# mrluin/TextualDegRemoval

Hardware: AMD Instinct MI355X
Metric: train images/sec (512x512, bs=4/GPU) (higher is better)
Workload: dtype f32 (3xbf16-split MFMA: 24-bit operand significands on the full fp32 exponent range, fp32 accumulate; unscaled gradients, no loss scale, no step-skip guard; tensors fp32 -- the MASA-encoder ResidualBlock activations / gradients as three bf16 planes whose sum IS the fp32 value, bit for bit)

## Files before the change

### include/tdr.h

```cpp
#ifndef TDR_H
#define TDR_H
#include <stdint.h>
#ifdef __cplusplus
extern "C" {
#endif

#define TDR_ABI_VERSION 112
int tdr_version(void);
const char* tdr_last_error(void);

typedef struct TdrStepGuard {
    float scale, inv_scale, max_scale;
    int good, growth_interval;
    int step, skipped, finite;
    float bc1, bc2_sqrt;
} TdrStepGuard;

typedef struct TdrConvDesc {
    int N, Cin, H, W;
    int Cout, OH, OW;
    int KH, stride, dil, pad;
    const float* in;  int64_t in_ns;
    int gate;
    const float* kscale; int64_t kscale_ns;
// ... 69 lines not shown
int64_t tdr_wgrad3x3_p16_ws_floats(const TdrWgradP16Desc* d);
int tdr_wgrad3x3_p16(const TdrWgradP16Desc* d, void* stream);

typedef struct TdrWgradDesc {
    int N, Cin, H, W, Cout, OH, OW, KH, stride, pad;
    const float* in;   int64_t in_ns;  int gate;
    const float* dout; int64_t dout_ns;
    float* g;
    float* db;
    int per_image;
    float* ws; int64_t ws_floats;
    int math;
} TdrWgradDesc;
int64_t tdr_wgrad_ws_floats(const TdrWgradDesc* d);
int tdr_conv_wgrad(const TdrWgradDesc* d, void* stream);

typedef struct TdrWg1GroupEntry {
    const float* in; const float* dout; float* part; float* dbpart; float* g; float* db;
} TdrWg1GroupEntry;
int tdr_wgrad1x1_group_supported(const TdrWgradDesc* d);
int64_t tdr_wgrad1x1_group_ws_floats(const TdrWgradDesc* d, int nprob);
int tdr_wgrad1x1_group(const TdrWgradDesc* d, int nprob, const void* table, void* stream);

int64_t tdr_wgrad3x3_p16_group_ws_floats(const TdrWgradP16Desc* d, int nprob);
int tdr_wgrad3x3_p16_group_plan(const TdrWgradP16Desc* d, int nprob, int* nsplit, int* units, int* units_per_wg);
int tdr_wgrad3x3_p16_group(const TdrWgradP16Desc* d, int nprob, const void* table, void* stream);

int tdr_layernorm2d_fwd(const float* x, int64_t x_ns, const float* w, const float* b, float eps, int center,
                        int N, int C, int HW, float* y, float* mu, float* rstd, void* stream);
int64_t tdr_ln_ws_floats(int N, int C, int HW);
// ... 36 lines not shown
int tdr_mdta_pad(int C);
int tdr_mdta_softmax(const float* G, const float* ss, const float* temp, int N, int C, int heads, float* A, float* AT,
                     void* stream);
int tdr_mdta_bwd(const float* G, const float* ss, const float* temp, const float* A, const float* dA, int N, int C,
                 int heads, float* W, float* dtemp, float* ws, void* stream);
int tdr_attn_fold_proj(const float* AT, const float* Wo, int N, int C, int heads, float* Wf, void* stream);
int tdr_axpby_dev(const float* a, const float* alpha, const float* b, int64_t numel, float* out, void* stream);
int tdr_dot(const float* a, const float* b, int64_t numel, float* out, float* ws, void* stream);
int tdr_pixel_shuffle2(const float* in, int N, int C, int H, int W, float* out, void* stream);

int tdr_sca_fwd(const float* pooled, const float* wsca, const float* bsca, int N, int C, float* s, void* stream);
int tdr_sca_bwd(const float* G3, const float* S3, const float* w3, const float* b3, const float* beta,
                const float* s, const float* pooled, const float* wsca, int N, int C,
                float* dw3, float* db3, float* dbeta, float* dwsca, float* dbsca, float* dpooled,
                float* ws , void* stream);
int tdr_scaled_conv_param_grads(const float* G, const float* S, const float* w, const float* b,
                                const float* gamma, int Cout, int Cin, float* dw, float* db, float* dgamma,
                                void* stream);

int64_t tdr_chansum_ws_floats(int N, int C, int HW);
int tdr_channel_sum(const float* x, int64_t x_ns, int N, int C, int HW, float* out, float* ws, void* stream);

int tdr_copy_rows(const float* src, int64_t src_ns, float* dst, int64_t dst_ns, int N, int64_t len, void* stream);
int tdr_add_rows(const float* src, int64_t src_ns, float* dst, int64_t dst_ns, int N, int64_t len, void* stream);
int tdr_pixel_unshuffle2(const float* in, int N, int C, int H, int W, float* out, void* stream);
int tdr_pad_crop(const float* src, int N, int C, int Hs, int Ws, float* dst, int Hd, int Wd, void* stream);
int tdr_crop_augment(const float* src, int64_t src_ns, int N, int C, int Hs, int Ws, const int* top, const int* left,
                     const int* mode, const float* noise, const float* sigma, int P, float* out, void* stream);

int64_t tdr_ssim3d_ws_floats(int H, int W);
// ... 363 lines not shown
```

### textualdegremoval_amd/csrc/tdr_pointwise.hip

```cpp
#include "tdr_common.h"
#include "../../include/tdr.h"

namespace {

template <int SLICES, int CPT>
__global__ __launch_bounds__(64 * SLICES) void ln_fwd_kernel(const float* __restrict__ x, long x_ns,
                                                            const float* __restrict__ w, const float* __restrict__ b,
                                                            float eps, int center, int C, int HW,
                                                            float* __restrict__ y, float* __restrict__ mu,
                                                            float* __restrict__ rstd) {
    __shared__ float red[SLICES][64];
    const int lane = threadIdx.x & 63, slice = threadIdx.x >> 6;
    const int px = blockIdx.x * 64 + lane, n = blockIdx.y;
    const bool pok = px < HW;
    const float* xn = x + (long)n * x_ns + (pok ? px : HW - 1);
    float v[CPT];
    float s = 0.f;
#pragma unroll
    for (int i = 0; i < CPT; ++i) v[i] = xn[(long)min(slice + SLICES * i, C - 1) * HW];
#pragma unroll
    for (int i = 0; i < CPT; ++i) {
        v[i] = (pok && slice + SLICES * i < C) ? v[i] : 0.f;
        s += v[i];
    }
// ... 546 lines not shown
            if (n == 0) {
                float sb = 0.f;
                for (int m = 0; m < N; ++m) sb += ds[(long)m * C + cj];
                dbsca[cj] = sb;
            }
        }
        return;
    }
    const int colb = (C + 255) / 256;
    const int r = (int)blockIdx.x - ntail;
    const int ci = (r / colb) * 4 + (threadIdx.x >> 8), cj = (r % colb) * 256 + (threadIdx.x & 255);
    if (ci >= C || cj >= C) return;
    float a = 0.f;
    for (int n = 0; n < N; ++n) a += ds[(long)n * C + ci] * pooled[(long)n * C + cj];
    dwsca[(long)ci * C + cj] = a;
}

__global__ __launch_bounds__(256) void scaled_conv_param_kernel(const float* __restrict__ G, const float* __restrict__ S,
                                                               const float* __restrict__ w, const float* __restrict__ b,
                                                               const float* __restrict__ gamma, int Cin,
                                                               float* __restrict__ dw, float* __restrict__ db,
                                                               float* __restrict__ dgamma) {
    __shared__ float red[4];
    const int co = blockIdx.x;
    const float gm = gamma[co];
    float acc = 0.f;
    for (int ci = threadIdx.x; ci < Cin; ci += 256) {
        const float gv = G[(long)co * Cin + ci];
        dw[(long)co * Cin + ci] = gm * gv;
        acc += w[(long)co * Cin + ci] * gv;
// ... 376 lines not shown
        hipLaunchKernelGGL(sca_bwd_rows_kernel, dim3(C), dim3(256), 0, st, G3, S3, w3, b3, beta, s, N, C, dw3, db3, dbeta);
        hipLaunchKernelGGL(sca_bwd_ds_kernel, dim3(tdr_cdiv(C, 64), N), dim3(1024), 0, st, G3, w3, beta, N, C, ds);
        hipLaunchKernelGGL(sca_bwd_dw_kernel, dim3(tdr_cdiv(C, 256), C), dim3(256), 0, st, ds, pooled, N, C, dwsca);
        hipLaunchKernelGGL(sca_bwd_tail_kernel, dim3(tdr_cdiv(C, 64), N), dim3(1024), 0, st, ds, wsca, N, C, dbsca, dpooled);
    } else {
        const int nt = tdr_cdiv(C, 64) * N;
        hipLaunchKernelGGL(sca_bwd_a_kernel, dim3(nt + tdr_cdiv(C, 4)), dim3(1024), 0, st, G3, S3, w3, b3, beta, s, N, C, nt, dw3,
                           db3, dbeta, ds);
        hipLaunchKernelGGL(sca_bwd_b_kernel, dim3(nt + tdr_cdiv(C, 4) * tdr_cdiv(C, 256)), dim3(1024), 0, st, ds, pooled, wsca, N, C,
                           nt, dwsca, dbsca, dpooled);
    }
    TDR_LAUNCH_CHECK("sca_bwd");
    return TDR_OK;
}

extern "C" int tdr_scaled_conv_param_grads(const float* G, const float* S, const float* w, const float* b,
                                           const float* gamma, int Cout, int Cin, float* dw, float* db, float* dgamma,
                                           void* stream) {
    TDR_REQUIRE(G && S && w && b && gamma && dw && db && dgamma, "tdr_scaled_conv_param_grads: null pointer");
    hipLaunchKernelGGL(scaled_conv_param_kernel, dim3(Cout), dim3(256), 0, (hipStream_t)stream, G, S, w, b, gamma, Cin, dw,
                       db, dgamma);
    TDR_LAUNCH_CHECK("scaled_conv_param_kernel");
    return TDR_OK;
}

extern "C" int64_t tdr_chansum_ws_floats(int N, int C, int HW) {
    (void)N; (void)HW;
    return (int64_t)C * CS_SPLITS;
}

// ... 164 lines not shown
```

### textualdegremoval_amd/csrc/tdr_wgrad_1x1.hip

```cpp
#include "tdr_common.h"
#include "tdr_wgrad_common.h"
#include "../../include/tdr.h"
#include <stdlib.h>

typedef __bf16 g1bf16x8 __attribute__((ext_vector_type(8)));
typedef _Float16 g1f16x8 __attribute__((ext_vector_type(8)));
typedef unsigned g1u32x4 __attribute__((ext_vector_type(4)));

namespace {

enum { G1_BX3 = 0, G1_HX2 = 1 };

constexpr int G1_PX = 32;

template <int SCH>
__device__ __forceinline__ void g1_split8(const f32x4& a, const f32x4& b, g1u32x4 (&p)[SCH == G1_BX3 ? 3 : 2]) {
    if constexpr (SCH == G1_BX3) {
        unsigned h[4], m[4], l[4];
        tdr_split3_bf16<false>(a[0], a[1], h[0], m[0], l[0]);
        tdr_split3_bf16<false>(a[2], a[3], h[1], m[1], l[1]);
        tdr_split3_bf16<false>(b[0], b[1], h[2], m[2], l[2]);
        tdr_split3_bf16<false>(b[2], b[3], h[3], m[3], l[3]);
        p[0] = (g1u32x4){h[0], h[1], h[2], h[3]};
        p[1] = (g1u32x4){m[0], m[1], m[2], m[3]};
// ... 179 lines not shown
    constexpr size_t lds = (size_t)RING * (BM + (GATE ? 2 : 1) * BN) * 128;
    static_assert(lds <= 160 * 1024, "LDS");
    dim3 grid(N * a.spi, tdr_cdiv(a.Cout, BM), tdr_cdiv(a.Cin, BN));
    auto kern = wgrad1x1_dma_kernel<TMW, TNW, GATE, SCH, RING>;
    static bool attr_set = false;
    if (!attr_set) {
        (void)hipFuncSetAttribute(reinterpret_cast<const void*>(kern), hipFuncAttributeMaxDynamicSharedMemorySize, 160 * 1024);
        attr_set = true;
    }
    hipLaunchKernelGGL(kern, grid, dim3(256), lds, st, a);
    TDR_LAUNCH_CHECK("wgrad1x1_dma_kernel");
    return TDR_OK;
}


template <bool GATE, int SCH, int KQ, bool GRP = false, int TNW = 2, int TMW = 2>
__global__ __launch_bounds__(256 * KQ) void wgrad1x1_sp_kernel(WgArgs a) {
    static_assert(KQ == 1 || TMW == 2, "the in-block K split is built for 128-row tiles");
    constexpr int BM = 64 * TMW, BN = 64 * TNW, NI = TMW + TNW;
    constexpr int NS = SCH == G1_BX3 ? 3 : 2, NP = SCH == G1_BX3 ? 6 : 3;
    constexpr int ROWS = BM + BN;
    constexpr int PLANE = ROWS * 32;
    constexpr int KSTR = NS * PLANE + 64;
    constexpr int BUF = KQ * KSTR;
    constexpr int PXS = 16 * KQ;
    constexpr int NL = GATE ? NI + TNW : NI;

    extern __shared__ __attribute__((aligned(1024))) unsigned char smem_raw[];
    const int tid = threadIdx.x, lane = tid & 63, wave = __builtin_amdgcn_readfirstlane(tid >> 6);
    const int kq = KQ == 2 ? wave >> 2 : 0, wm = (wave >> 1) & 1, wn = wave & 1;
    const int j = lane & 31, kg = lane >> 5;

    int prob = 0, split = blockIdx.x, by = blockIdx.y, bz = blockIdx.z;
// ... 136 lines not shown
        split_store(raw0, 0, s + 2 < nst);
        interleave();
        __syncthreads();
    }

    if (want_db) {
#pragma unroll
        for (int i = 0; i < TMW; ++i) {
            float t = dsum[i];
            t += __shfl_xor(t, 1, 64); t += __shfl_xor(t, 2, 64);
            if constexpr (KQ == 2) t += __shfl_xor(t, 4, 64);
            const int co = co0 + lr + 64 * i;
            if (lp == 0 && co < a.Cout) a.dbpart[(long)split * a.Cout + co] = t;
        }
    }
    float* red = reinterpret_cast<float*>(smem_raw);
    const int wq = wave & 3;
    if (KQ == 2 && kq == 1) {
#pragma unroll
        for (int x = 0; x < TMW; ++x)
#pragma unroll
            for (int y = 0; y < TNW; ++y)
#pragma unroll
                for (int r = 0; r < 16; ++r) red[((wq * 4 + x * 2 + y) * 16 + r) * 64 + lane] = acc[x][y][r];
    }
    if constexpr (KQ == 2) {
        __syncthreads();
        if (kq == 1) return;
    }
    float* part = a.part + (long)split * a.Cout * a.Cin;
// ... 11 lines not shown
        }
}

template <bool GATE, int SCH, int KQ>
int launch_sp(const WgArgs& a, int N, hipStream_t st) {
    constexpr int NS = SCH == G1_BX3 ? 3 : 2;
    constexpr size_t lds0 = (size_t)2 * KQ * (NS * 256 * 32 + 64);
    constexpr size_t lds = (KQ == 2 && lds0 < 65536) ? 65536 : lds0;
    dim3 grid(N * a.spi, tdr_cdiv(a.Cout, 128), tdr_cdiv(a.Cin, 128));
    auto kern = wgrad1x1_sp_kernel<GATE, SCH, KQ>;
    static bool attr_set = false;
    if (!attr_set) {
        (void)hipFuncSetAttribute(reinterpret_cast<const void*>(kern), hipFuncAttributeMaxDynamicSharedMemorySize, 160 * 1024);
        attr_set = true;
    }
    hipLaunchKernelGGL(kern, grid, dim3(256 * KQ), lds, st, a);
    TDR_LAUNCH_CHECK("wgrad1x1_sp_kernel");
    return TDR_OK;
}

int g1_sp() {
    static const int v = tdr_tune_env("TDR_WG1_SP") ? atoi(tdr_tune_env("TDR_WG1_SP")) : 2;
    return v;
}

int g1_ring() {
    static const int r = tdr_tune_env("TDR_WG1_RING") ? atoi(tdr_tune_env("TDR_WG1_RING")) : 2;
    return r == 3 ? 3 : 2;
}

template <int TMW, int TNW, int SCH>
int launch_g1_gr(const WgArgs& a, const TdrWgradDesc* d, hipStream_t st) {
// ... 49 lines not shown

template <bool GATE, int SCH, int TNW, int TMW>
int launch_grp(const WgArgs& a, int nprob, hipStream_t st) {
    constexpr int NS = SCH == G1_BX3 ? 3 : 2;
    constexpr size_t lds0 = (size_t)2 * (NS * (64 * TMW + 64 * TNW) * 32 + 64);
    static const size_t pad = tdr_tune_env("TDR_WG1_GRP_LDS") ? (size_t)atol(tdr_tune_env("TDR_WG1_GRP_LDS")) : 0;
    const size_t lds = lds0 < pad ? pad : lds0;
    const int T = a.tiles_x * a.tiles_y;
    dim3 grid((unsigned)tdr_cdiv(a.grp_pairs, 8) * 8 * T);
    auto kern = wgrad1x1_sp_kernel<GATE, SCH, 1, true, TNW, TMW>;
    static bool attr_set = false;
    if (!attr_set) {
        (void)hipFuncSetAttribute(reinterpret_cast<const void*>(kern), hipFuncAttributeMaxDynamicSharedMemorySize, 160 * 1024);
        attr_set = true;
    }
    hipLaunchKernelGGL(kern, grid, dim3(256), lds, st, a);
    TDR_LAUNCH_CHECK("wgrad1x1_sp_kernel<grouped>");
    return TDR_OK;
}

}

extern "C" int tdr_wgrad1x1_group_supported(const TdrWgradDesc* d) {
    if (!d || (d->math != 1 && d->math != 2) || d->per_image) return 0;
    if (d->KH != 1 || d->stride != 1 || d->pad != 0 || d->H != d->OH || d->W != d->OW) return 0;
    const long HW = (long)d->OH * d->OW;
    if (HW % G1_PX != 0 || d->in_ns % 4 != 0 || d->dout_ns % 4 != 0) return 0;
    return d->Cin >= 64 && d->Cout > 64;
}

extern "C" int64_t tdr_wgrad1x1_group_ws_floats(const TdrWgradDesc* d, int nprob) {
// ... 70 lines not shown

int tdr_wgrad_1x1_launch(const WgArgs& a, const WgPlan& p, const TdrWgradDesc* d, hipStream_t st) {
    if (p.cfg == 0 && g1_sp() == 1) {
        const bool g = d->gate != 0;
        if (a.scheme == 1) return g ? launch_sp<true, G1_HX2, 2>(a, d->N, st) : launch_sp<false, G1_HX2, 2>(a, d->N, st);
        return g ? launch_sp<true, G1_BX3, 2>(a, d->N, st) : launch_sp<false, G1_BX3, 2>(a, d->N, st);
    }
    if (p.cfg == 0 && g1_sp() == 2) {
        const bool g = d->gate != 0;
        if (a.scheme == 1) return g ? launch_sp<true, G1_HX2, 1>(a, d->N, st) : launch_sp<false, G1_HX2, 1>(a, d->N, st);
        return g ? launch_sp<true, G1_BX3, 1>(a, d->N, st) : launch_sp<false, G1_BX3, 1>(a, d->N, st);
    }
    if (a.scheme == 1) return p.cfg == 0 ? launch_g1_gr<2, 2, G1_HX2>(a, d, st) : launch_g1_gr<1, 1, G1_HX2>(a, d, st);
    return p.cfg == 0 ? launch_g1_gr<2, 2, G1_BX3>(a, d, st) : launch_g1_gr<1, 1, G1_BX3>(a, d, st);
}
```

### textualdegremoval_amd/csrc/tdr_wgrad_common.h

```cpp
#pragma once
#include "tdr_common.h"

struct TdrWgradDesc;

struct WgArgs {
    const float* in; long in_ns; int Cin, H, W; long gate_off;
    const float* dout; long dout_ns; int Cout, OH, OW;
    int pad, tw_log2, tiles_x, tiles_y, tpi , tps , spi ;
    float* part;
    float* dbpart;
    int scheme;
    const void* grp_tab;
    int grp_bpp;
    int grp_pairs;
};

struct WgPlan { int tw_log2, tiles_x, tiles_y, tpi, tps, spi, cfg, WKw, BMc, BNc; };

bool tdr_wgrad_bx3_supported(const TdrWgradDesc* d);
WgPlan tdr_wgrad_bx3_plan(const TdrWgradDesc* d);
int tdr_wgrad_bx3_launch(const WgArgs& a, const WgPlan& p, const TdrWgradDesc* d, hipStream_t st);

bool tdr_wgrad_s2_supported(const TdrWgradDesc* d);
WgPlan tdr_wgrad_s2_plan(const TdrWgradDesc* d);
int tdr_wgrad_s2_launch(const WgArgs& a, const WgPlan& p, const TdrWgradDesc* d, hipStream_t st);

bool tdr_wgrad_1x1_supported(const TdrWgradDesc* d);
WgPlan tdr_wgrad_1x1_plan(const TdrWgradDesc* d);
int tdr_wgrad_1x1_launch(const WgArgs& a, const WgPlan& p, const TdrWgradDesc* d, hipStream_t st);
```

### textualdegremoval_amd/csrc/tdr_wgrad_mfma.hip

```cpp
#include <stdio.h>
#include <stdlib.h>
#include "tdr_common.h"
#include "tdr_wgrad_common.h"
#include "../../include/tdr.h"

namespace {

constexpr int wg_plane(int TW, int KH, int S) { return (((64 / TW) - 1) * S + KH) * ((TW - 1) * S + KH); }
constexpr int wg_cmax(int a, int b) { return a > b ? a : b; }
constexpr int wg_max_plane(int KH, int S) {
    return wg_cmax(wg_plane(8, KH, S), wg_cmax(wg_plane(16, KH, S), wg_plane(32, KH, S)));
}

template <int KH, int S, int WMw, int WNw, int WKw, int TMW, int TNW, bool GATE>
__global__ __launch_bounds__(256) void wgrad_mfma_kernel(WgArgs a) {
    static_assert(WMw * WNw * WKw == 4, "4 waves");
    constexpr int TAPS = KH * KH;
    constexpr int BMc = 32 * TMW * WMw, BNc = 32 * TNW * WNw;
    constexpr int MAXPIT = (wg_max_plane(KH, S) + 63) / 64;
    constexpr int DPT = BMc / 4;
    constexpr int IPT = BNc / 4;
    constexpr int KPW = 32 / WKw;

    extern __shared__ __attribute__((aligned(16))) float smem[];
// ... 217 lines not shown
    const int TW = 1 << a.tw_log2;
    const int LH = ((64 >> a.tw_log2) - 1) * S + KH, LW = (TW - 1) * S + KH;
    const size_t lds = (size_t)(BMc * 65 + BNc * ((LH * LW) | 1)) * sizeof(float);
    dim3 grid(N * p.spi, tdr_cdiv(a.Cout, BMc), tdr_cdiv(a.Cin, BNc));
    auto kern = wgrad_mfma_kernel<KH, S, WMw, WNw, WKw, TMW, TNW, GATE>;
    static bool attr_set = false;
    if (!attr_set) {
        (void)hipFuncSetAttribute(reinterpret_cast<const void*>(kern), hipFuncAttributeMaxDynamicSharedMemorySize, 160 * 1024);
        attr_set = true;
    }
    hipLaunchKernelGGL(kern, grid, dim3(256), lds, st, a);
    TDR_LAUNCH_CHECK("wgrad_mfma_kernel");
    return TDR_OK;
}

}

extern "C" int64_t tdr_wgrad_ws_floats(const TdrWgradDesc* d) {
    const WgPlan p = make_plan(d);
    return (int64_t)d->N * p.spi * p.WKw * d->Cout * d->Cin * d->KH * d->KH + (int64_t)d->N * p.spi * d->Cout;
}

extern "C" int tdr_conv_wgrad(const TdrWgradDesc* d, void* stream) {
    TDR_REQUIRE(d && d->in && d->dout && d->g && d->ws, "tdr_conv_wgrad: null pointer");
    const WgPlan p = make_plan(d);
    const int64_t need = tdr_wgrad_ws_floats(d);
    TDR_REQUIRE(d->ws_floats >= need, "tdr_conv_wgrad: workspace too small (%lld < %lld)", (long long)d->ws_floats,
                (long long)need);
    WgArgs a;
    a.in = d->in; a.in_ns = d->in_ns; a.Cin = d->Cin; a.H = d->H; a.W = d->W;
    a.gate_off = (long)d->Cin * d->H * d->W;
    a.dout = d->dout; a.dout_ns = d->dout_ns; a.Cout = d->Cout; a.OH = d->OH; a.OW = d->OW;
    a.grp_tab = nullptr; a.grp_bpp = 0; a.grp_pairs = 0;
    a.pad = d->pad; a.tw_log2 = p.tw_log2; a.tiles_x = p.tiles_x; a.tiles_y = p.tiles_y; a.tpi = p.tpi; a.tps = p.tps; a.spi = p.spi;
    const bool direct = !d->db && (d->per_image ? p.spi : d->N * p.spi) * p.WKw == 1;
    a.part = direct ? d->g : d->ws;
    a.dbpart = d->db ? d->ws + (int64_t)d->N * p.spi * p.WKw * d->Cout * d->Cin * d->KH * d->KH : nullptr;
    hipStream_t st = (hipStream_t)stream;
    const bool g = d->gate != 0;
    int rc = TDR_ERR_UNSUPPORTED;
    const int key = d->KH * 10 + d->stride;
    a.scheme = d->math == 3 ? 2 : (d->math == 2 ? 1 : 0);
    static const bool dbg = tdr_tune_env("TDR_WG_DEBUG") != nullptr;
    if (dbg && !(d->math >= 1 && tdr_wgrad_bx3_supported(d)) && !tdr_wgrad_s2_supported(d))
        fprintf(stderr, "[tdr] exact wgrad: math %d N %d %d->%d @%dx%d k%d s%d pad %d gate %d per_image %d in_ns %ld dout_ns %ld\n", d->math,
                d->N, d->Cin, d->Cout, d->H, d->W, d->KH, d->stride, d->pad, d->gate, d->per_image, (long)d->in_ns, (long)d->dout_ns);
    if (tdr_wgrad_1x1_supported(d)) {
        rc = tdr_wgrad_1x1_launch(a, p, d, st);
    } else if (d->math >= 1 && tdr_wgrad_bx3_supported(d)) {
        rc = tdr_wgrad_bx3_launch(a, p, d, st);
    } else if (tdr_wgrad_s2_supported(d)) {
        rc = tdr_wgrad_s2_launch(a, p, d, st);
    } else if (key == 11) {
        switch (p.cfg) {
            case 0: rc = g ? launch_wg<1, 1, 2, 2, 1, 2, 2, true>(a, p, d->N, st) : launch_wg<1, 1, 2, 2, 1, 2, 2, false>(a, p, d->N, st); break;
            case 1: rc = g ? launch_wg<1, 1, 1, 1, 4, 2, 1, true>(a, p, d->N, st) : launch_wg<1, 1, 1, 1, 4, 2, 1, false>(a, p, d->N, st); break;
            case 2: rc = g ? launch_wg<1, 1, 2, 2, 1, 1, 1, true>(a, p, d->N, st) : launch_wg<1, 1, 2, 2, 1, 1, 1, false>(a, p, d->N, st); break;
            default: rc = g ? launch_wg<1, 1, 1, 1, 4, 1, 1, true>(a, p, d->N, st) : launch_wg<1, 1, 1, 1, 4, 1, 1, false>(a, p, d->N, st); break;
        }
    } else if (key == 31 && !g) {
        rc = p.cfg == 3 ? launch_wg<3, 1, 1, 1, 4, 1, 1, false>(a, p, d->N, st) : launch_wg<3, 1, 2, 2, 1, 1, 1, false>(a, p, d->N, st);
    } else if (key == 32 && !g) {
        rc = launch_wg<3, 2, 2, 2, 1, 1, 1, false>(a, p, d->N, st);
    } else if (key == 22 && !g) {
        rc = launch_wg<2, 2, 2, 2, 1, 1, 1, false>(a, p, d->N, st);
    } else {
        tdr_set_error("tdr_conv_wgrad: unsupported (KH=%d stride=%d gate=%d)", d->KH, d->stride, d->gate);
        return TDR_ERR_UNSUPPORTED;
    }
    if (rc != TDR_OK || direct) return rc;
    const long elems = (long)d->Cout * d->Cin * d->KH * d->KH;
    const int groups = d->per_image ? d->N : 1;
    const int per_group = (d->per_image ? p.spi : d->N * p.spi) * p.WKw;
    const int nb_main = tdr_cdiv(elems, 64);
    const int nb2 = d->db ? tdr_cdiv(d->Cout, 64) : 0;
    const int pg2 = d->N * p.spi;
    const dim3 rgrid(nb_main + nb2, groups);
    if (per_group <= 8 && pg2 <= 8)
        hipLaunchKernelGGL(wgrad_reduce_kernel<1>, rgrid, dim3(64), 0, st, d->ws, elems, per_group, d->g, nb_main, a.dbpart,
                           (long)d->Cout, pg2, d->db);
    else if (per_group <= 64 && pg2 <= 64)
        hipLaunchKernelGGL(wgrad_reduce_kernel<4>, rgrid, dim3(256), 0, st, d->ws, elems, per_group, d->g, nb_main, a.dbpart,
                           (long)d->Cout, pg2, d->db);
    else
        hipLaunchKernelGGL(wgrad_reduce_kernel<16>, rgrid, dim3(1024), 0, st, d->ws, elems, per_group, d->g, nb_main, a.dbpart,
                           (long)d->Cout, pg2, d->db);
    TDR_LAUNCH_CHECK("wgrad_reduce_kernel");
    return TDR_OK;
}
```

### textualdegremoval_amd/engine.py

```python
import contextlib
import os
import types

import torch

from . import kernels as K
from . import leaves as L
from .kernels import (EPI_GATEBWD, EPI_PSHUF, PACK_DGRAD_2X2S2, PACK_DGRAD_3X3S2, PACK_DGRAD_S1, PACK_FWD)

LN_EPS = 1e-6
FUSE_TAIL = True
FUSE_HEAD = True
FUSE_CONV3_DGRAD = True
INFER_KERNELS = True
LOCAL_KERNELS = True


def _sub(P, pre):
    n = len(pre)
    return {k[n:]: v for k, v in P.items() if k.startswith(pre)}


def _put(G, pre, g):
    for k, v in g.items():
        G[pre + k] = v


DEFER_WGRAD = True
# ... 105 lines not shown
        else:
            dy, dt4, gw2, gb2 = K.naf_tail_bwd(dout, gamma, t4, y, mu2, rs2, P['norm2.weight'], w5t, w4t, defer_finish=late)
        if late:
            L.leaf_fin(('norm2.weight', 'norm2.bias'), gw2, G)
        else:
            G['norm2.weight'], G['norm2.bias'] = gw2, gb2
    else:
        wp, mp, *_ = K.pack_weights(P['conv5.weight'][:c_out], PACK_DGRAD_S1)
        dt4 = K.conv_forward(dout, wp, mp, c, 1, epi=EPI_GATEBWD, kscale=gamma, aux=t4)
    L.leaf_wgrad1x1((yn, dt4), (yn, dt4, 2 * c, c, False),
                    lambda g4, b4: {'conv4.weight': g4.view(2 * c, c, 1, 1), 'conv4.bias': b4}, G)
    if not fused:
        wp, mp, *_ = K.pack_weights(P['conv4.weight'], PACK_DGRAD_S1)
        dyn = K.conv_forward(dt4, wp, mp, c, 1)
        dy, G['norm2.weight'], G['norm2.bias'] = K.layernorm2d_bwd(dyn, y, mu2, rs2, P['norm2.weight'], add=dout)
    G3, S3 = K.conv_wgrad(g, dy, c, c, 1, per_image=True, want_db=True)
    dw3, db3, dbeta, dwsca, dbsca, dpooled = K.sca_bwd(G3, S3, P['conv3.weight'], P['conv3.bias'], beta, s, pooled,
                                                       P['sca.1.weight'])
    G['conv3.weight'], G['conv3.bias'], G['beta'] = dw3, db3, dbeta
    G['sca.1.weight'], G['sca.1.bias'] = dwsca, dbsca
    if fused and FUSE_CONV3_DGRAD:
        dt1, gdw, gdb = K.dwsg_bwd(dgp, t1, P['conv2.weight'], P['conv2.bias'], dg_bias=dpooled, dg_bias_mul=1.0 / (H * W),
                                   defer_finish=late)
    else:
        wp, mp, *_ = K.pack_weights(P['conv3.weight'], PACK_DGRAD_S1)
        dg = K.conv_forward(dy, wp, mp, c, 1, kscale=beta, scale=s, bias2=dpooled, bias2_mul=1.0 / (H * W))
        dt1, gdw, gdb = K.dwsg_bwd(dg, t1, P['conv2.weight'], P['conv2.bias'], defer_finish=late)
    if isinstance(gdw, K.Finisher):
        L.leaf_fin(('conv2.weight', 'conv2.bias'), gdw, G)
    else:
        G['conv2.weight'], G['conv2.bias'] = gdw, gdb
    L.leaf_wgrad1x1((xn, dt1), (xn, dt1, 2 * c, c, False),
                    lambda g1, b1: {'conv1.weight': g1.view(2 * c, c, 1, 1), 'conv1.bias': b1}, G)
    if FUSE_TAIL and K.naf_tail_supported(c, H * W) and _dgrad_fused_ok() and x.is_contiguous() and dy.is_contiguous():
# ... 537 lines not shown
```

### textualdegremoval_amd/kernels.py

```python
import contextlib
import ctypes as C
import os

import torch

from . import _lib
from ._lib import TdrConvDesc, TdrConvP16Desc, TdrWgradDesc, TdrWgradP16Desc, check

EPI_STD, EPI_GATEBWD, EPI_PSHUF = 0, 1, 2
PACK_FWD, PACK_DGRAD_S1, PACK_DGRAD_2X2S2, PACK_DGRAD_3X3S2 = 0, 1, 2, 3

MATH = os.environ.get('TDR_MATH', 'bx3')
WGRAD_1X1_BX3 = True
FMT_F32, FMT_BX3, FMT_HX2, FMT_H1 = 0, 1, 2, 3


def fp16_path():
    return MATH in ('hx2', 'h1')


GRAD_SCALED = False
BACKWARD_PHASE = False


# ... 549 lines not shown
    d.g = g.data_ptr()
    db = torch.empty(Cout, dtype=torch.float32, device=x.device) if want_db else None
    d.db = _p(db)
    d.per_image = 1 if per_image else 0
    if fp16_path() and (fp16_range or GRAD_SCALED) and (KH == 3 or WGRAD_1X1_BX3):
        d.math = 2 if MATH == 'hx2' else 3
    else:
        d.math = 1 if (MATH != 'f32' and (KH == 3 or WGRAD_1X1_BX3)) else 0
    if _survey is not None and d.math >= 2:
        _survey.probe(dout, 'fwd' if fp16_range else 'grad')
    need = lib.tdr_wgrad_ws_floats(C.byref(d))
    ws = workspace(need, x.device, 'wgrad')
    d.ws, d.ws_floats = ws.data_ptr(), ws.numel()
    check(lib.tdr_conv_wgrad(C.byref(d), _stream()), 'tdr_conv_wgrad')
    return (g, db) if want_db else g


def _wgrad1x1_desc(x, dout, Cout, Cin, gate):
    N, _, H, W = x.shape
    d = TdrWgradDesc()
    d.N, d.Cin, d.H, d.W, d.Cout, d.OH, d.OW = N, Cin, H, W, Cout, H, W
    d.KH, d.stride, d.pad = 1, 1, 0
    d.in_ns, d.gate, d.dout_ns = _dense_nchw(x), 1 if gate else 0, _dense_nchw(dout)
    d.per_image = 0
    if fp16_path() and GRAD_SCALED and WGRAD_1X1_BX3:
        d.math = 2 if MATH == 'hx2' else 3
    else:
        d.math = 1 if (MATH != 'f32' and WGRAD_1X1_BX3) else 0
    return d

# ... 434 lines not shown
    N, Cc = s.shape
    dev = s.device
    dw3 = torch.empty(Cc, Cc, 1, 1, dtype=torch.float32, device=dev)
    db3 = torch.empty(Cc, dtype=torch.float32, device=dev)
    dbeta = torch.empty(1, Cc, 1, 1, dtype=torch.float32, device=dev)
    dwsca = torch.empty(Cc, Cc, 1, 1, dtype=torch.float32, device=dev)
    dbsca = torch.empty(Cc, dtype=torch.float32, device=dev)
    dpooled = torch.empty(N, Cc, dtype=torch.float32, device=dev)
    ws = torch.empty(N * Cc, dtype=torch.float32, device=dev)
    check(lib.tdr_sca_bwd(G3.data_ptr(), S3.data_ptr(), w3.data_ptr(), b3.data_ptr(), beta.data_ptr(), s.data_ptr(),
                          pooled.data_ptr(), wsca.data_ptr(), N, Cc, dw3.data_ptr(), db3.data_ptr(), dbeta.data_ptr(),
                          dwsca.data_ptr(), dbsca.data_ptr(), dpooled.data_ptr(), ws.data_ptr(), _stream()), 'tdr_sca_bwd')
    return dw3, db3, dbeta, dwsca, dbsca, dpooled


def scaled_conv_param_grads(G, S, w, b, gamma):
    lib = _lib.load()
    Cout, Cin = G.shape[-2], G.shape[-1]
    dev = G.device
    dw = torch.empty(Cout, Cin, dtype=torch.float32, device=dev)
    db = torch.empty(Cout, dtype=torch.float32, device=dev)
    dg = torch.empty(Cout, dtype=torch.float32, device=dev)
    check(lib.tdr_scaled_conv_param_grads(G.data_ptr(), S.data_ptr(), w.data_ptr(), b.data_ptr(), gamma.data_ptr(), Cout,
                                          Cin, dw.data_ptr(), db.data_ptr(), dg.data_ptr(), _stream()),
          'tdr_scaled_conv_param_grads')
    return dw, db, dg


def channel_sum(x):
    lib = _lib.load()
# ... 1388 lines not shown
```

Before: 61.89.

## Fold SCA ds into conv3 Gram wgrad epilogue and defer Gram reduction

The per-image 1x1 conv3 weight-gradient kernel gains an epilogue that forms partial ds sums (beta·w3·Gram tile) directly from its accumulators. A new SCA backward kernel then reduces those partials into ds, dwsca, dbsca and dpooled without waiting for the full Gram reduction. The Gram reduce and the conv3/beta parameter-gradient kernels move into a deferred leaf finisher, taking them off the critical path of the activation-gradient chain. The cost is extra register and LDS work in the wgrad epilogue, an extra partials buffer and an added kernel variant.

```diff
diff --git a/include/tdr.h b/include/tdr.h
--- a/include/tdr.h
+++ b/include/tdr.h
@@ -107,6 +107,10 @@
 } TdrWgradDesc;
 int64_t tdr_wgrad_ws_floats(const TdrWgradDesc* d);
 int tdr_conv_wgrad(const TdrWgradDesc* d, void* stream);
+int tdr_wgrad_gram_ds_supported(const TdrWgradDesc* d);
+int tdr_wgrad_gram_ds_parts(const TdrWgradDesc* d);
+int tdr_wgrad_gram_ds(const TdrWgradDesc* d, const float* w3, const float* beta, float* dspart, void* stream);
+int tdr_wgrad_gram_finish(const TdrWgradDesc* d, void* stream);
 
 typedef struct TdrWg1GroupEntry {
     const float* in; const float* dout; float* part; float* dbpart; float* g; float* db;
@@ -173,6 +177,10 @@
                 const float* s, const float* pooled, const float* wsca, int N, int C,
                 float* dw3, float* db3, float* dbeta, float* dwsca, float* dbsca, float* dpooled,
                 float* ws , void* stream);
+int tdr_sca_bwd_parts(const float* dspart, int nk, const float* pooled, const float* wsca, int N, int C, float* ds,
+                      float* dwsca, float* dbsca, float* dpooled, void* stream);
+int tdr_sca_bwd_rows(const float* G3, const float* S3, const float* w3, const float* b3, const float* beta, const float* s,
+                     int N, int C, float* dw3, float* db3, float* dbeta, void* stream);
 int tdr_scaled_conv_param_grads(const float* G, const float* S, const float* w, const float* b,
                                 const float* gamma, int Cout, int Cin, float* dw, float* db, float* dgamma,
                                 void* stream);
diff --git a/textualdegremoval_amd/csrc/tdr_pointwise.hip b/textualdegremoval_amd/csrc/tdr_pointwise.hip
--- a/textualdegremoval_amd/csrc/tdr_pointwise.hip
+++ b/textualdegremoval_amd/csrc/tdr_pointwise.hip
@@ -584,6 +584,82 @@
     float a = 0.f;
     for (int n = 0; n < N; ++n) a += ds[(long)n * C + ci] * pooled[(long)n * C + cj];
     dwsca[(long)ci * C + cj] = a;
+}
+
+__device__ __forceinline__ float sca_fold_run(const float* __restrict__ p, int C, int k0, int k1) {
+    float t = 0.f;
+    for (int k = k0; k < k1; k += 8) {
+        float v[8];
+#pragma unroll
+        for (int u = 0; u < 8; ++u) v[u] = k + u < k1 ? p[(long)(k + u) * C] : 0.f;
+#pragma unroll
+        for (int u = 0; u < 8; ++u) t += v[u];
+    }
+    return t;
+}
+
+constexpr int SCA_PARTS_MAXC = 1024;
+
+__global__ __launch_bounds__(1024) void sca_bwd_bp_kernel(const float* __restrict__ dspart, int nk, int G, int kper,
+                                                         const float* __restrict__ pooled, const float* __restrict__ wsca, int N, int C,
+                                                         int ntail, float* __restrict__ ds, float* __restrict__ dwsca,
+                                                         float* __restrict__ dbsca, float* __restrict__ dpooled) {
+    __shared__ float red[16][64];
+    __shared__ float runs[SCA_PARTS_MAXC];
+    __shared__ float dsl[SCA_PARTS_MAXC];
+    const int tid = threadIdx.x;
+    if ((int)blockIdx.x < ntail) {
+        const int tiles = (C + 63) / 64;
+        const int tile = blockIdx.x % tiles, n = blockIdx.x / tiles;
+        const int g = tid / C, ci = tid - g * C;
+        if (g < G) runs[tid] = sca_fold_run(dspart + (long)n * nk * C + ci, C, g * kper, min(nk, (g + 1) * kper));
+        __syncthreads();
+        if (tid < C) {
+            float t = 0.f;
+            for (int q = 0; q < G; ++q) t += runs[q * C + tid];
+            dsl[tid] = t;
+            if (tile == 0) ds[(long)n * C + tid] = t;
+        }
+        __syncthreads();
+        const int lane = tid & 63, sl = tid >> 6;
+        const int cj = tile * 64 + lane;
+        const int cjc = min(cj, C - 1);
+        float a = 0.f;
+        for (int c = sl; c < C; c += 16) a += wsca[(long)c * C + cjc] * dsl[c];
+        red[sl][lane] = a;
+        __syncthreads();
+        if (sl == 0 && cj < C) {
+            float t = 0.f;
+#pragma unroll
+            for (int q = 0; q < 16; ++q) t += red[q][lane];
+            dpooled[(long)n * C + cj] = t;
+        }
+        return;
+    }
+    const int colb = (C + 255) / 256;
+    const int r = (int)blockIdx.x - ntail;
+    const int ci0 = (r / colb) * 4, sub = tid >> 8;
+    if (tid < 4 * N * G) {
+        const int v = tid / G, g = tid - v * G;
+        const int cic = min(ci0 + v / N, C - 1);
+        runs[tid] = sca_fold_run(dspart + (long)(v % N) * nk * C + cic, C, g * kper, min(nk, (g + 1) * kper));
+    }
+    __syncthreads();
+    if (tid < 4 * N) {
+        float t = 0.f;
+        for (int q = 0; q < G; ++q) t += runs[tid * G + q];
+        dsl[tid] = t;
+    }
+    __syncthreads();
+    const int ci = ci0 + sub, cj = (r % colb) * 256 + (tid & 255);
+    if (ci >= C || cj >= C) return;
+    float a = 0.f, sb = 0.f;
+    for (int n = 0; n < N; ++n) {
+        a += dsl[sub * N + n] * pooled[(long)n * C + cj];
+        sb += dsl[sub * N + n];
+    }
+    dwsca[(long)ci * C + cj] = a;
+    if (cj == 0) dbsca[ci] = sb;
 }
 
 __global__ __launch_bounds__(256) void scaled_conv_param_kernel(const float* __restrict__ G, const float* __restrict__ S,
@@ -990,6 +1066,30 @@
     return TDR_OK;
 }
 
+extern "C" int tdr_sca_bwd_parts(const float* dspart, int nk, const float* pooled, const float* wsca, int N, int C, float* ds,
+                                 float* dwsca, float* dbsca, float* dpooled, void* stream) {
+    TDR_REQUIRE(dspart && pooled && wsca && ds && dwsca && dbsca && dpooled, "tdr_sca_bwd_parts: null pointer");
+    TDR_REQUIRE(nk > 0 && N > 0 && N <= 256 && C > 0 && C <= SCA_PARTS_MAXC, "tdr_sca_bwd_parts: need 0 < N <= 256, 0 < C <= %d, nk > 0", SCA_PARTS_MAXC);
+    int G = SCA_PARTS_MAXC / C;
+    if (G > 256 / N) G = 256 / N;
+    if (G > nk) G = nk;
+    const int kper = tdr_cdiv(nk, G);
+    const int nt = tdr_cdiv(C, 64) * N;
+    hipLaunchKernelGGL(sca_bwd_bp_kernel, dim3(nt + tdr_cdiv(C, 4) * tdr_cdiv(C, 256)), dim3(1024), 0, (hipStream_t)stream, dspart, nk, G, kper,
+                       pooled, wsca, N, C, nt, ds, dwsca, dbsca, dpooled);
+    TDR_LAUNCH_CHECK("sca_bwd_parts");
+    return TDR_OK;
+}
+
+extern "C" int tdr_sca_bwd_rows(const float* G3, const float* S3, const float* w3, const float* b3, const float* beta, const float* s,
+                                int N, int C, float* dw3, float* db3, float* dbeta, void* stream) {
+    TDR_REQUIRE(G3 && S3 && w3 && b3 && beta && s && dw3 && db3 && dbeta, "tdr_sca_bwd_rows: null pointer");
+    hipLaunchKernelGGL(sca_bwd_a_kernel, dim3(tdr_cdiv(C, 4)), dim3(1024), 0, (hipStream_t)stream, G3, S3, w3, b3, beta, s, N, C, 0, dw3, db3,
+                       dbeta, static_cast<float*>(nullptr));
+    TDR_LAUNCH_CHECK("sca_bwd_rows");
+    return TDR_OK;
+}
+
 extern "C" int tdr_scaled_conv_param_grads(const float* G, const float* S, const float* w, const float* b,
                                            const float* gamma, int Cout, int Cin, float* dw, float* db, float* dgamma,
                                            void* stream) {
diff --git a/textualdegremoval_amd/csrc/tdr_wgrad_1x1.hip b/textualdegremoval_amd/csrc/tdr_wgrad_1x1.hip
--- a/textualdegremoval_amd/csrc/tdr_wgrad_1x1.hip
+++ b/textualdegremoval_amd/csrc/tdr_wgrad_1x1.hip
@@ -217,9 +217,10 @@
 }
 
 
-template <bool GATE, int SCH, int KQ, bool GRP = false, int TNW = 2, int TMW = 2>
-__global__ __launch_bounds__(256 * KQ) void wgrad1x1_sp_kernel(WgArgs a) {
+template <bool GATE, int SCH, int KQ, bool GRP = false, int TNW = 2, int TMW = 2, bool DSP = false>
+__global__ __launch_bounds__(256 * KQ) void wgrad1x1_sp_kernel(WgArgs a, G1DsArgs e) {
     static_assert(KQ == 1 || TMW == 2, "the in-block K split is built for 128-row tiles");
+    static_assert(!DSP || (KQ == 1 && !GRP && !GATE && TNW == 2 && TMW == 2), "the ds-partial epilogue: plain 128 x 128 tiles, no in-block K split");
     constexpr int BM = 64 * TMW, BN = 64 * TNW, NI = TMW + TNW;
     constexpr int NS = SCH == G1_BX3 ? 3 : 2, NP = SCH == G1_BX3 ? 6 : 3;
     constexpr int ROWS = BM + BN;
@@ -386,6 +387,36 @@
             if (lp == 0 && co < a.Cout) a.dbpart[(long)split * a.Cout + co] = t;
         }
     }
+    if constexpr (DSP) {
+        float* fold = reinterpret_cast<float*>(smem_raw);
+        float* bl = fold + 256;
+        if (tid < 128) bl[tid] = co0 + tid < a.Cout ? e.beta[co0 + tid] : 0.f;
+        float wv[TNW][TMW][16];
+#pragma unroll
+        for (int y = 0; y < TNW; ++y) {
+            const int cic = min(ci0 + (wn * TNW + y) * 32 + j, a.Cin - 1);
+#pragma unroll
+            for (int x = 0; x < TMW; ++x)
+#pragma unroll
+                for (int r = 0; r < 16; ++r) {
+                    const int co = min(co0 + (wm * TMW + x) * 32 + (r & 3) + 8 * (r >> 2) + 4 * kg, a.Cout - 1);
+                    wv[y][x][r] = *reinterpret_cast<const float*>(reinterpret_cast<const char*>(e.w3) + 4u * (unsigned)(co * a.Cin + cic));
+                }
+        }
+        __syncthreads();
+#pragma unroll
+        for (int y = 0; y < TNW; ++y) {
+            float t = 0.f;
+#pragma unroll
+            for (int x = 0; x < TMW; ++x)
+#pragma unroll
+                for (int r = 0; r < 16; ++r) t += bl[(wm * TMW + x) * 32 + (r & 3) + 8 * (r >> 2) + 4 * kg] * wv[y][x][r] * acc[x][y][r];
+            t += __shfl_xor(t, 32, 64);
+            if (kg == 0) fold[wm * 128 + (wn * TNW + y) * 32 + j] = t;
+        }
+        __syncthreads();
+        if (tid < 128 && ci0 + tid < a.Cin) e.dspart[((long)split * gridDim.y + by) * a.Cin + ci0 + tid] = fold[tid] + fold[128 + tid];
+    }
     float* red = reinterpret_cast<float*>(smem_raw);
     const int wq = wave & 3;
     if (KQ == 2 && kq == 1) {
@@ -427,8 +458,24 @@
         (void)hipFuncSetAttribute(reinterpret_cast<const void*>(kern), hipFuncAttributeMaxDynamicSharedMemorySize, 160 * 1024);
         attr_set = true;
     }
-    hipLaunchKernelGGL(kern, grid, dim3(256 * KQ), lds, st, a);
+    hipLaunchKernelGGL(kern, grid, dim3(256 * KQ), lds, st, a, G1DsArgs{nullptr, nullptr, nullptr});
     TDR_LAUNCH_CHECK("wgrad1x1_sp_kernel");
+    return TDR_OK;
+}
+
+template <int SCH>
+int launch_sp_ds(const WgArgs& a, const G1DsArgs& e, int N, hipStream_t st) {
+    constexpr int NS = SCH == G1_BX3 ? 3 : 2;
+    constexpr size_t lds = (size_t)2 * (NS * 256 * 32 + 64);
+    dim3 grid(N * a.spi, tdr_cdiv(a.Cout, 128), tdr_cdiv(a.Cin, 128));
+    auto kern = wgrad1x1_sp_kernel<false, SCH, 1, false, 2, 2, true>;
+    static bool attr_set = false;
+    if (!attr_set) {
+        (void)hipFuncSetAttribute(reinterpret_cast<const void*>(kern), hipFuncAttributeMaxDynamicSharedMemorySize, 160 * 1024);
+        attr_set = true;
+    }
+    hipLaunchKernelGGL(kern, grid, dim3(256), lds, st, a, e);
+    TDR_LAUNCH_CHECK("wgrad1x1_sp_kernel<ds partials>");
     return TDR_OK;
 }
 
@@ -508,7 +555,7 @@
         (void)hipFuncSetAttribute(reinterpret_cast<const void*>(kern), hipFuncAttributeMaxDynamicSharedMemorySize, 160 * 1024);
         attr_set = true;
     }
-    hipLaunchKernelGGL(kern, grid, dim3(256), lds, st, a);
+    hipLaunchKernelGGL(kern, grid, dim3(256), lds, st, a, G1DsArgs{nullptr, nullptr, nullptr});
     TDR_LAUNCH_CHECK("wgrad1x1_sp_kernel<grouped>");
     return TDR_OK;
 }
@@ -609,3 +656,12 @@
     if (a.scheme == 1) return p.cfg == 0 ? launch_g1_gr<2, 2, G1_HX2>(a, d, st) : launch_g1_gr<1, 1, G1_HX2>(a, d, st);
     return p.cfg == 0 ? launch_g1_gr<2, 2, G1_BX3>(a, d, st) : launch_g1_gr<1, 1, G1_BX3>(a, d, st);
 }
+
+bool tdr_wgrad_1x1_ds_supported(const TdrWgradDesc* d) {
+    return tdr_wgrad_1x1_supported(d) && d->Cout > 64 && d->Cin > 64 && !d->gate && g1_sp() == 2;
+}
+
+int tdr_wgrad_1x1_launch_ds(const WgArgs& a, const WgPlan& p, const TdrWgradDesc* d, const G1DsArgs& e, hipStream_t st) {
+    if (p.cfg != 0 || !tdr_wgrad_1x1_ds_supported(d)) return TDR_ERR_UNSUPPORTED;
+    return a.scheme == 1 ? launch_sp_ds<G1_HX2>(a, e, d->N, st) : launch_sp_ds<G1_BX3>(a, e, d->N, st);
+}
diff --git a/textualdegremoval_amd/csrc/tdr_wgrad_common.h b/textualdegremoval_amd/csrc/tdr_wgrad_common.h
--- a/textualdegremoval_amd/csrc/tdr_wgrad_common.h
+++ b/textualdegremoval_amd/csrc/tdr_wgrad_common.h
@@ -17,6 +17,8 @@
 
 struct WgPlan { int tw_log2, tiles_x, tiles_y, tpi, tps, spi, cfg, WKw, BMc, BNc; };
 
+struct G1DsArgs { const float* w3; const float* beta; float* dspart; };
+
 bool tdr_wgrad_bx3_supported(const TdrWgradDesc* d);
 WgPlan tdr_wgrad_bx3_plan(const TdrWgradDesc* d);
 int tdr_wgrad_bx3_launch(const WgArgs& a, const WgPlan& p, const TdrWgradDesc* d, hipStream_t st);
@@ -28,3 +30,5 @@
 bool tdr_wgrad_1x1_supported(const TdrWgradDesc* d);
 WgPlan tdr_wgrad_1x1_plan(const TdrWgradDesc* d);
 int tdr_wgrad_1x1_launch(const WgArgs& a, const WgPlan& p, const TdrWgradDesc* d, hipStream_t st);
+bool tdr_wgrad_1x1_ds_supported(const TdrWgradDesc* d);
+int tdr_wgrad_1x1_launch_ds(const WgArgs& a, const WgPlan& p, const TdrWgradDesc* d, const G1DsArgs& e, hipStream_t st);
diff --git a/textualdegremoval_amd/csrc/tdr_wgrad_mfma.hip b/textualdegremoval_amd/csrc/tdr_wgrad_mfma.hip
--- a/textualdegremoval_amd/csrc/tdr_wgrad_mfma.hip
+++ b/textualdegremoval_amd/csrc/tdr_wgrad_mfma.hip
@@ -255,6 +255,40 @@
     return TDR_OK;
 }
 
+WgArgs wg_args(const TdrWgradDesc* d, const WgPlan& p, bool direct) {
+    WgArgs a;
+    a.in = d->in; a.in_ns = d->in_ns; a.Cin = d->Cin; a.H = d->H; a.W = d->W;
+    a.gate_off = (long)d->Cin * d->H * d->W;
+    a.dout = d->dout; a.dout_ns = d->dout_ns; a.Cout = d->Cout; a.OH = d->OH; a.OW = d->OW;
+    a.grp_tab = nullptr; a.grp_bpp = 0; a.grp_pairs = 0;
+    a.pad = d->pad; a.tw_log2 = p.tw_log2; a.tiles_x = p.tiles_x; a.tiles_y = p.tiles_y; a.tpi = p.tpi; a.tps = p.tps; a.spi = p.spi;
+    a.part = direct ? d->g : d->ws;
+    a.dbpart = d->db ? d->ws + (int64_t)d->N * p.spi * p.WKw * d->Cout * d->Cin * d->KH * d->KH : nullptr;
+    a.scheme = d->math == 3 ? 2 : (d->math == 2 ? 1 : 0);
+    return a;
+}
+
+int wg_reduce(const TdrWgradDesc* d, const WgPlan& p, const float* dbpart, hipStream_t st) {
+    const long elems = (long)d->Cout * d->Cin * d->KH * d->KH;
+    const int groups = d->per_image ? d->N : 1;
+    const int per_group = (d->per_image ? p.spi : d->N * p.spi) * p.WKw;
+    const int nb_main = tdr_cdiv(elems, 64);
+    const int nb2 = d->db ? tdr_cdiv(d->Cout, 64) : 0;
+    const int pg2 = d->N * p.spi;
+    const dim3 rgrid(nb_main + nb2, groups);
+    if (per_group <= 8 && pg2 <= 8)
+        hipLaunchKernelGGL(wgrad_reduce_kernel<1>, rgrid, dim3(64), 0, st, d->ws, elems, per_group, d->g, nb_main, dbpart,
+                           (long)d->Cout, pg2, d->db);
+    else if (per_group <= 64 && pg2 <= 64)
+        hipLaunchKernelGGL(wgrad_reduce_kernel<4>, rgrid, dim3(256), 0, st, d->ws, elems, per_group, d->g, nb_main, dbpart,
+                           (long)d->Cout, pg2, d->db);
+    else
+        hipLaunchKernelGGL(wgrad_reduce_kernel<16>, rgrid, dim3(1024), 0, st, d->ws, elems, per_group, d->g, nb_main, dbpart,
+                           (long)d->Cout, pg2, d->db);
+    TDR_LAUNCH_CHECK("wgrad_reduce_kernel");
+    return TDR_OK;
+}
+
 }
 
 extern "C" int64_t tdr_wgrad_ws_floats(const TdrWgradDesc* d) {
@@ -268,20 +302,12 @@
     const int64_t need = tdr_wgrad_ws_floats(d);
     TDR_REQUIRE(d->ws_floats >= need, "tdr_conv_wgrad: workspace too small (%lld < %lld)", (long long)d->ws_floats,
                 (long long)need);
-    WgArgs a;
-    a.in = d->in; a.in_ns = d->in_ns; a.Cin = d->Cin; a.H = d->H; a.W = d->W;
-    a.gate_off = (long)d->Cin * d->H * d->W;
-    a.dout = d->dout; a.dout_ns = d->dout_ns; a.Cout = d->Cout; a.OH = d->OH; a.OW = d->OW;
-    a.grp_tab = nullptr; a.grp_bpp = 0; a.grp_pairs = 0;
-    a.pad = d->pad; a.tw_log2 = p.tw_log2; a.tiles_x = p.tiles_x; a.tiles_y = p.tiles_y; a.tpi = p.tpi; a.tps = p.tps; a.spi = p.spi;
     const bool direct = !d->db && (d->per_image ? p.spi : d->N * p.spi) * p.WKw == 1;
-    a.part = direct ? d->g : d->ws;
-    a.dbpart = d->db ? d->ws + (int64_t)d->N * p.spi * p.WKw * d->Cout * d->Cin * d->KH * d->KH : nullptr;
+    const WgArgs a = wg_args(d, p, direct);
     hipStream_t st = (hipStream_t)stream;
     const bool g = d->gate != 0;
     int rc = TDR_ERR_UNSUPPORTED;
     const int key = d->KH * 10 + d->stride;
-    a.scheme = d->math == 3 ? 2 : (d->math == 2 ? 1 : 0);
     static const bool dbg = tdr_tune_env("TDR_WG_DEBUG") != nullptr;
     if (dbg && !(d->math >= 1 && tdr_wgrad_bx3_supported(d)) && !tdr_wgrad_s2_supported(d))
         fprintf(stderr, "[tdr] exact wgrad: math %d N %d %d->%d @%dx%d k%d s%d pad %d gate %d per_image %d in_ns %ld dout_ns %ld\n", d->math,
@@ -310,22 +336,32 @@
         return TDR_ERR_UNSUPPORTED;
     }
     if (rc != TDR_OK || direct) return rc;
-    const long elems = (long)d->Cout * d->Cin * d->KH * d->KH;
-    const int groups = d->per_image ? d->N : 1;
-    const int per_group = (d->per_image ? p.spi : d->N * p.spi) * p.WKw;
-    const int nb_main = tdr_cdiv(elems, 64);
-    const int nb2 = d->db ? tdr_cdiv(d->Cout, 64) : 0;
-    const int pg2 = d->N * p.spi;
-    const dim3 rgrid(nb_main + nb2, groups);
-    if (per_group <= 8 && pg2 <= 8)
-        hipLaunchKernelGGL(wgrad_reduce_kernel<1>, rgrid, dim3(64), 0, st, d->ws, elems, per_group, d->g, nb_main, a.dbpart,
-                           (long)d->Cout, pg2, d->db);
-    else if (per_group <= 64 && pg2 <= 64)
-        hipLaunchKernelGGL(wgrad_reduce_kernel<4>, rgrid, dim3(256), 0, st, d->ws, elems, per_group, d->g, nb_main, a.dbpart,
-                           (long)d->Cout, pg2, d->db);
-    else
-        hipLaunchKernelGGL(wgrad_reduce_kernel<16>, rgrid, dim3(1024), 0, st, d->ws, elems, per_group, d->g, nb_main, a.dbpart,
-                           (long)d->Cout, pg2, d->db);
-    TDR_LAUNCH_CHECK("wgrad_reduce_kernel");
-    return TDR_OK;
-}
+    return wg_reduce(d, p, a.dbpart, st);
+}
+
+extern "C" int tdr_wgrad_gram_ds_supported(const TdrWgradDesc* d) {
+    return d && d->per_image && tdr_wgrad_1x1_ds_supported(d) ? 1 : 0;
+}
+
+extern "C" int tdr_wgrad_gram_ds_parts(const TdrWgradDesc* d) {
+    if (!tdr_wgrad_gram_ds_supported(d)) return 0;
+    return make_plan(d).spi * tdr_cdiv(d->Cout, 128);
+}
+
+extern "C" int tdr_wgrad_gram_ds(const TdrWgradDesc* d, const float* w3, const float* beta, float* dspart, void* stream) {
+    TDR_REQUIRE(d && d->in && d->dout && d->ws && d->db && w3 && beta && dspart, "tdr_wgrad_gram_ds: null pointer");
+    TDR_REQUIRE(tdr_wgrad_gram_ds_supported(d), "tdr_wgrad_gram_ds: not a per-image 1x1 Gram with a bias gradient on the split-once kernel");
+    const WgPlan p = make_plan(d);
+    TDR_REQUIRE(d->ws_floats >= tdr_wgrad_ws_floats(d), "tdr_wgrad_gram_ds: workspace too small (%lld < %lld)", (long long)d->ws_floats,
+                (long long)tdr_wgrad_ws_floats(d));
+    const WgArgs a = wg_args(d, p, false);
+    const G1DsArgs e = {w3, beta, dspart};
+    return tdr_wgrad_1x1_launch_ds(a, p, d, e, (hipStream_t)stream);
+}
+
+extern "C" int tdr_wgrad_gram_finish(const TdrWgradDesc* d, void* stream) {
+    TDR_REQUIRE(d && d->g && d->db && d->ws, "tdr_wgrad_gram_finish: null pointer");
+    TDR_REQUIRE(tdr_wgrad_gram_ds_supported(d), "tdr_wgrad_gram_finish: not a launch of tdr_wgrad_gram_ds");
+    const WgPlan p = make_plan(d);
+    return wg_reduce(d, p, wg_args(d, p, false).dbpart, (hipStream_t)stream);
+}
diff --git a/textualdegremoval_amd/engine.py b/textualdegremoval_amd/engine.py
--- a/textualdegremoval_amd/engine.py
+++ b/textualdegremoval_amd/engine.py
@@ -12,6 +12,7 @@
 FUSE_TAIL = True
 FUSE_HEAD = True
 FUSE_CONV3_DGRAD = True
+SCA_PARTIALS = True
 INFER_KERNELS = True
 LOCAL_KERNELS = True
 
@@ -147,10 +148,15 @@
         wp, mp, *_ = K.pack_weights(P['conv4.weight'], PACK_DGRAD_S1)
         dyn = K.conv_forward(dt4, wp, mp, c, 1)
         dy, G['norm2.weight'], G['norm2.bias'] = K.layernorm2d_bwd(dyn, y, mu2, rs2, P['norm2.weight'], add=dout)
-    G3, S3 = K.conv_wgrad(g, dy, c, c, 1, per_image=True, want_db=True)
-    dw3, db3, dbeta, dwsca, dbsca, dpooled = K.sca_bwd(G3, S3, P['conv3.weight'], P['conv3.bias'], beta, s, pooled,
-                                                       P['sca.1.weight'])
-    G['conv3.weight'], G['conv3.bias'], G['beta'] = dw3, db3, dbeta
+    if SCA_PARTIALS and K.conv3_gram_ds_supported(g, dy, c):
+        dspart, fin3 = K.conv3_gram_ds(g, dy, P['conv3.weight'], P['conv3.bias'], beta, s)
+        _ds, dwsca, dbsca, dpooled = K.sca_bwd_parts(dspart, pooled, P['sca.1.weight'])
+        L.leaf_fin(('conv3.weight', 'conv3.bias', 'beta'), fin3, G)
+    else:
+        G3, S3 = K.conv_wgrad(g, dy, c, c, 1, per_image=True, want_db=True)
+        dw3, db3, dbeta, dwsca, dbsca, dpooled = K.sca_bwd(G3, S3, P['conv3.weight'], P['conv3.bias'], beta, s, pooled,
+                                                           P['sca.1.weight'])
+        G['conv3.weight'], G['conv3.bias'], G['beta'] = dw3, db3, dbeta
     G['sca.1.weight'], G['sca.1.bias'] = dwsca, dbsca
     if fused and FUSE_CONV3_DGRAD:
         dt1, gdw, gdb = K.dwsg_bwd(dgp, t1, P['conv2.weight'], P['conv2.bias'], dg_bias=dpooled, dg_bias_mul=1.0 / (H * W),
diff --git a/textualdegremoval_amd/kernels.py b/textualdegremoval_amd/kernels.py
--- a/textualdegremoval_amd/kernels.py
+++ b/textualdegremoval_amd/kernels.py
@@ -587,6 +587,57 @@
     d.ws, d.ws_floats = ws.data_ptr(), ws.numel()
     check(lib.tdr_conv_wgrad(C.byref(d), _stream()), 'tdr_conv_wgrad')
     return (g, db) if want_db else g
+
+
+def _gram_ds_desc(x, dout, Cc):
+    N, _, H, W = x.shape
+    d = TdrWgradDesc()
+    d.N, d.Cin, d.H, d.W, d.Cout, d.OH, d.OW = N, Cc, H, W, Cc, H, W
+    d.KH, d.stride, d.pad = 1, 1, 0
+    d.inp, d.in_ns, d.gate = x.data_ptr(), _dense_nchw(x), 0
+    d.dout, d.dout_ns = dout.data_ptr(), _dense_nchw(dout)
+    d.per_image = 1
+    if fp16_path() and GRAD_SCALED and WGRAD_1X1_BX3:
+        d.math = 2 if MATH == 'hx2' else 3
+    else:
+        d.math = 1 if (MATH != 'f32' and WGRAD_1X1_BX3) else 0
+    return d
+
+
+def conv3_gram_ds_supported(x, dout, Cc):
+    if x.shape != dout.shape or x.shape[1] != Cc or Cc > 1024 or x.shape[0] > 256:
+        return False
+    return bool(_lib.load().tdr_wgrad_gram_ds_supported(C.byref(_gram_ds_desc(x, dout, Cc))))
+
+
+def conv3_gram_ds(x, dout, w3, b3, beta, s):
+    lib = _lib.load()
+    N, Cc, H, W = x.shape
+    dev = x.device
+    d = _gram_ds_desc(x, dout, Cc)
+    if _survey is not None and d.math >= 2:
+        _survey.probe(dout, 'grad')
+    nk = int(lib.tdr_wgrad_gram_ds_parts(C.byref(d)))
+    assert nk > 0, 'conv3_gram_ds: shape not supported (see conv3_gram_ds_supported)'
+    S3 = torch.empty(Cc, dtype=torch.float32, device=dev)
+    d.db = S3.data_ptr()
+    ws = torch.empty(int(lib.tdr_wgrad_ws_floats(C.byref(d))), dtype=torch.float32, device=dev)
+    d.ws, d.ws_floats = ws.data_ptr(), ws.numel()
+    dspart = torch.empty(N, nk, Cc, dtype=torch.float32, device=dev)
+    check(lib.tdr_wgrad_gram_ds(C.byref(d), w3.data_ptr(), beta.data_ptr(), dspart.data_ptr(), _stream()), 'tdr_wgrad_gram_ds')
+
+    def fin():
+        G3 = torch.empty(N, Cc, Cc, dtype=torch.float32, device=dev)
+        d.g = G3.data_ptr()
+        check(lib.tdr_wgrad_gram_finish(C.byref(d), _stream()), 'tdr_wgrad_gram_finish')
+        dw3 = torch.empty(Cc, Cc, 1, 1, dtype=torch.float32, device=dev)
+        db3 = torch.empty(Cc, dtype=torch.float32, device=dev)
+        dbeta = torch.empty(1, Cc, 1, 1, dtype=torch.float32, device=dev)
+        check(lib.tdr_sca_bwd_rows(G3.data_ptr(), S3.data_ptr(), w3.data_ptr(), b3.data_ptr(), beta.data_ptr(), s.data_ptr(), N, Cc,
+                                   dw3.data_ptr(), db3.data_ptr(), dbeta.data_ptr(), _stream()), 'tdr_sca_bwd_rows')
+        side_keep(G3, S3, ws)
+        return dw3, db3, dbeta
+    return dspart, Finisher(None, ws, (N, Cc), fin)
 
 
 def _wgrad1x1_desc(x, dout, Cout, Cin, gate):
@@ -1051,6 +1102,18 @@
     return dw3, db3, dbeta, dwsca, dbsca, dpooled
 
 
+def sca_bwd_parts(dspart, pooled, wsca):
+    N, nk, Cc = dspart.shape
+    dev = dspart.device
+    ds = torch.empty(N, Cc, dtype=torch.float32, device=dev)
+    dwsca = torch.empty(Cc, Cc, 1, 1, dtype=torch.float32, device=dev)
+    dbsca = torch.empty(Cc, dtype=torch.float32, device=dev)
+    dpooled = torch.empty(N, Cc, dtype=torch.float32, device=dev)
+    check(_lib.load().tdr_sca_bwd_parts(dspart.data_ptr(), nk, pooled.data_ptr(), wsca.data_ptr(), N, Cc, ds.data_ptr(), dwsca.data_ptr(),
+                                        dbsca.data_ptr(), dpooled.data_ptr(), _stream()), 'tdr_sca_bwd_parts')
+    return ds, dwsca, dbsca, dpooled
+
+
 def scaled_conv_param_grads(G, S, w, b, gamma):
     lib = _lib.load()
     Cout, Cin = G.shape[-2], G.shape[-1]
```

New measurement: 62.41, median of 6. Within noise of the previous version (+0.8%).
